# JinfengX/PointCloudPDF

Measured on AMD Instinct MI355X. Metric: points/sec fwd+bwd (PT-v1 Seg50 + PDF U-decoder, 100k-pt scenes), higher is better.
Workload: dtype f32

## Files before the change

### include/pdfops.h

```cpp
#ifndef PDFOPS_H
#define PDFOPS_H

#ifdef __cplusplus
extern "C" {
#endif

#define PDF_OK 0
#define PDF_ERR_BAD_ARG (-1)
#define PDF_ERR_NSAMPLE (-2)
#define PDF_ERR_UNSUPPORTED (-3)

#define PDF_ABI_VERSION 11
int pdf_abi_version(void);
const char *pdf_build_info(void);
int pdf_dist_fma_mode(void);
#define PDF_MMA_F32 0
#define PDF_MMA_F16 1
#define PDF_MMA_BF16 2

int pdf_knn_query(int m, int nsample, const float *xyz, const float *new_xyz,
                  const int *offset, const int *new_offset, int b,
                  int *idx, float *dist2, void *stream);

long pdf_knn_workspace_bytes(int b, int n, int m);
int pdf_knn_grid_supported(int nsample);
int pdf_knn_query_ws(int m, int nsample, int n, const float *xyz, const float *new_xyz, const int *offset,
                     const int *new_offset, int b, int *idx, float *dist2, void *workspace, long workspace_bytes,
                     void *stream);
int pdf_knn_grid_build(int n, const float *xyz, const int *offset, int b, void *workspace, long workspace_bytes, void *stream);
int pdf_knn_query_grid(int m, int nsample, int n, const float *xyz, const float *new_xyz, const int *offset, const int *new_offset, int b,
                       int *idx, float *dist2, void *workspace, long workspace_bytes, void *stream);
int pdf_knn_query_ws_counted(int m, int nsample, int n, const float *xyz, const float *new_xyz, const int *offset,
                             const int *new_offset, int b, int *idx, float *dist2, void *workspace, long workspace_bytes,
                             unsigned long long *pairs, void *stream);
int pdf_knn_query_list(int m, int nsample, const float *xyz, const float *new_xyz, const int *offset,
                       const int *new_offset, int b, int *idx, float *dist2, const int *qlist, const int *qcount,
                       void *stream);

int pdf_ball_query(int m, int nsample, float min_radius, float max_radius, const float *xyz, const float *new_xyz,
                   const int *offset, const int *new_offset, int b, int *idx, float *dist2, void *stream);

int pdf_random_ball_query(int m, int nsample, float min_radius, float max_radius, const int *order, const float *xyz,
                          const float *new_xyz, const int *offset, const int *new_offset, int b, int *idx, float *dist2,
                          void *stream);

int pdf_farthest_point_sampling(int b, int n, const float *xyz, const int *offset,
                                const int *new_offset, float *tmp, int *idx, void *stream);

int pdf_fps_reference_block_log2(int n);

long pdf_fps_workspace_bytes(int b, int n_total);
long pdf_fps_stats_offset(int b, int n_total);
int pdf_farthest_point_sampling_bucketed(int b, int n, int n_total, const float *xyz, const int *offset,
                                         const int *new_offset, void *workspace, long workspace_bytes,
                                         int *idx, void *stream);

int pdf_grouping_forward(int m, int nsample, int c, const float *input, const int *idx, float *output, void *stream);
int pdf_grouping_backward(int m, int nsample, int c, const float *grad_output, const int *idx, float *grad_input, void *stream);
int pdf_grouping_forward_ordered(int m, int nsample, int c, const float *input, const int *idx, const int *order, float *output, void *stream);
int pdf_group_forward_ordered(int m, int nsample, int c, int with_xyz, const float *feat, const float *xyz, const float *new_xyz,
                              const int *idx, const int *order, float *output, void *stream);
int pdf_interpolation_forward_ordered(int n, int c, int k, const float *input, const int *idx, const float *weight, const int *order,
                                      float *output, void *stream);
int pdf_subtraction_forward_ordered(int n, int nsample, int c, const float *input1, const float *input2, const int *idx, const int *order,
                                    float *output, void *stream);
int pdf_aggregation_forward_ordered(int n, int nsample, int c, int w_c, const float *input, const float *position, const float *weight,
                                    const int *idx, const int *order, float *output, void *stream);

int pdf_interpolation_forward(int n, int c, int k, const float *input, const int *idx, const float *weight, float *output, void *stream);
int pdf_interpolation_backward(int n, int c, int k, const float *grad_output, const int *idx, const float *weight, float *grad_input, void *stream);

int pdf_subtraction_forward(int n, int nsample, int c, const float *input1, const float *input2, const int *idx, float *output, void *stream);
int pdf_subtraction_backward(int n, int nsample, int c, const int *idx, const float *grad_output, float *grad_input1, float *grad_input2, void *stream);

int pdf_aggregation_forward(int n, int nsample, int c, int w_c, const float *input, const float *position,
                            const float *weight, const int *idx, float *output, void *stream);
int pdf_aggregation_backward(int n, int nsample, int c, int w_c, const float *input, const float *position,
                             const float *weight, const int *idx, const float *grad_output,
                             float *grad_input, float *grad_position, float *grad_weight, void *stream);

int pdf_attention_relation_step_forward(int m, int g, int c, const float *query, const float *key, const float *weight,
                                        const int *index_target, const int *index_refer, float *output, void *stream);
int pdf_attention_relation_step_backward(int m, int g, int c, const float *query, float *grad_query,
                                         const float *key, float *grad_key, const float *weight, float *grad_weight,
                                         const int *index_target, const int *index_refer, const float *grad_output, void *stream);
int pdf_attention_fusion_step_forward(int m, int g, int c, const float *weight, const float *value,
                                      const int *index_target, const int *index_refer, float *output, void *stream);
int pdf_attention_fusion_step_backward(int m, int g, int c, const float *weight, float *grad_weight,
                                       const float *value, float *grad_value,
                                       const int *index_target, const int *index_refer, const float *grad_output, void *stream);


int pdf_group_forward(int m, int nsample, int c, int with_xyz, const float *feat, const float *xyz,
                      const float *new_xyz, const int *idx, float *output, void *stream);
int pdf_group_backward(int m, int nsample, int c, int with_xyz, const float *grad_output, const int *idx,
                       float *grad_feat, void *stream);

int pdf_interpolation_weights(int n, int k, const float *dist2, float *weight, void *stream);

int pdf_pt_layer_supported(int nsample, int c);
long pdf_pt_layer_partial_floats(int n, int nsample, int c);
int pdf_pt_layer_forward(int n, int nsample, int c, const float *xq, const float *xk, const float *xv,
                         const float *p, const int *idx, const float *const *weights,
                         const float *const *bn_params, float *const *bn_buffers, int training, float eps,
                         float momentum, float *bn, float *saved, float *H, float *partial, float *out,
                         int storage_bf16, const int *order, void *stream);
int pdf_pt_layer_forward_m(int n, int nsample, int c, const float *xq, const float *xk, const float *xv,
                           const float *p, const int *idx, const float *const *weights,
                           const float *const *bn_params, float *const *bn_buffers, int training, float eps,
                           float momentum, float *bn, float *saved, float *H, float *partial, float *out,
                           int storage_bf16, const int *order, const double *moments, int *out_stat_rows, void *stream);

long pdf_pt_layer_bwd_partial_floats(int n, int nsample, int c);
long pdf_pt_layer_bwd_sums_floats(int c);
int pdf_pt_layer_backward(int n, int nsample, int c, const float *xq, const float *xk, const float *xv,
                          const float *p, const int *idx, const float *const *weights, const float *bn,
                          const float *saved, const float *H, const float *gout, float *gxq, float *gxk,
                          float *gxv, float *G2, float *G3, float *Wsm, float *GR, const int *inv_off, const int *inv_entry,
                          int entry_base, float *partial, float *sums, int storage_bf16, const int *order, const double *moments,
                          void *stream);

int pdf_bn_supported(int c);
long pdf_bn_partial_floats(long n, int c);
int pdf_bn_act_forward(long n, int c, const float *x, const float *res, const float *gamma, const float *beta,
                       float *running_mean, float *running_var, int training, float eps, float momentum, int relu,
                       float *coef, float *partial, float *y, void *stream);
int pdf_bn_act_backward(long n, int c, const float *gy, const float *x, const float *res, const float *coef,
                        int training, int relu, float *partial, float *sums, float *gx, float *gres, void *stream);
int pdf_bn_coef(long n, int c, const float *x, const float *gamma, const float *beta, float *running_mean,
                float *running_var, int training, float eps, float momentum, float *coef, float *partial, void *stream);
int pdf_bn_apply(long n, int c, const float *x, const float *res, const float *coef, int relu, float *y, void *stream);

long pdf_rowlin_partial_floats(long n, int o);
int pdf_rowlin_partial_rows(long n, int k, int o);
int pdf_rowlin_forward(long n, int k, int o, const float *x, long ldx, const float *w, int transpose_w,
                       const float *bias, const float *scale, const float *shift, int relu, float *y, long ldy,
                       int accumulate, float *partial, int mma_input, void *stream);
long pdf_rowlin_wgrad_ws_floats(long n, int k, int o, int ng);
int pdf_rowlin_wgrad(long n, int k, int o, const float *g, long ldg, const float *x, long ldx,
                     const float *scale, const float *shift, int relu, float *dw, float *db, float *ws, int mma_input, void *stream);
int pdf_bn_coef_from_partial(const float *partial, int rows, long n, int c, const float *gamma, const float *beta,
                             float *running_mean, float *running_var, float eps, float momentum, float *coef, void *stream);

int pdf_rowlin_multi(long n, int k, int o, int nin, int nout, const float *const *x, long ldx, const float *const *w,
                     int transpose_w, const float *const *bias, const float *scale, const float *shift, int relu,
                     float *const *y, long ldy, int accumulate, int mma_input, void *stream);
int pdf_rowlin_wgrad_multi(long n, int k, int o, int ng, const float *const *g, long ldg, const float *x, long ldx,
                           const float *scale, const float *shift, int relu, float *const *dw, float *const *db, float *ws, int mma_input, void *stream);
int pdf_rowlin_wgrad_group(long n, int k, int o, int ng, const float *const *g, long ldg, const float *const *x, long ldx,
                           const float *const *scale, const float *const *shift, const int *relu, float *const *dw,
                           float *const *db, float *ws, int mma_input, void *stream);

int pdf_kpconv_supported(int kp, int cin);
int pdf_kpconv_gather(int n, int m, int kp, int cin, const float *query, const float *support, const int *neighbors, const float *x,
                      const float *k_points, float extent, float *weighted, void *stream);
int pdf_kpconv_scatter(int n, int m, int kp, int cin, const float *query, const float *support, const int *neighbors,
                       const float *grad_weighted, const float *k_points, float extent, float *grad_x, void *stream);
int pdf_rowlin_dgrad_bstats(long n, int k, int o, int nin, const float *const *x, long ldx, const float *const *w, float *y, long ldy,
                            const float *bx, long ldb, const float *bcoef, int brelu, float *partial, int *partial_rows,
                            int mma_input, void *stream);
int pdf_rowlin_forward_bn(long n, int k, int o, const float *x, long ldx, const float *w, const float *bias, const float *scale,
                          const float *shift, int relu, float *y, long ldy, float *partial, const float *gamma, const float *beta,
                          float *running_mean, float *running_var, float eps, float momentum, float *coef, int mma_input, void *stream);
int pdf_bn_act_backward_presummed(long n, int c, const float *gy, const float *x, const float *coef, int training, int relu,
                                  const float *partial, int partial_rows, float *sums, float *gx, void *stream);

int pdf_bn_coef_eval_or_partial(const float *partial, int rows, long n, int c, const float *gamma, const float *beta,
                                float *running_mean, float *running_var, int training, float eps, float momentum,
                                float *coef, void *stream);
int pdf_block_pre_forward(long n, int c, void *const *p, int training, float eps, float momentum, int mma_input, void *stream);
int pdf_block_pre_backward(long n, int c, void *const *p, int training, int mma_input, void *stream);
int pdf_block_post_forward(long n, int c, void *const *p, int training, float eps, float momentum, int mma_input, void *stream);
int pdf_block_post_backward(long n, int c, void *const *p, int training, int mma_input, void *stream);
int pdf_bottleneck_forward(long n, int nsample, int c, void *const *p, int training, float eps, float momentum, int storage_bf16, int mma_input, void *stream);
int pdf_bottleneck_backward(long n, int nsample, int c, void *const *p, int training, int entry_base, int storage_bf16, int mma_input, void *stream);
int pdf_linbn_forward(long n, int k, int o, void *const *p, int training, int relu, float eps, float momentum, int mma_input, void *stream);
int pdf_linbn_backward(long n, int k, int o, void *const *p, int training, int relu, int mma_input, void *stream);

int pdf_rowlin_forward_roww(long n, int k, int o, const float *x, long ldx, const float *w, int transpose_w, float *y, long ldy,
                            int accumulate, const float *roww, long rws, int mma_input, void *stream);
int pdf_rowlin_wgrad_roww(long n, int k, int o, const float *g, long ldg, const float *x, long ldx, float *dw, const float *roww,
                          long rws, float *ws, int mma_input, void *stream);
int pdf_bn_bwd_sums(long n, int c, const float *gy, const float *x, const float *coef, int relu, float *partial, float *sums,
                    void *stream);

int pdf_td_supported(int nsample, int cin, int cout);
int pdf_td_tables(long m, int b, const float *p_src, const float *p_new, const int *idx, const int *new_offset, float *rel4, float *Z,
                  float *scene_sums, long n, const int *inv_off, const int *inv_entry, int entry_base,
                  void *stream);
long pdf_td_gram_floats(int cin);
long pdf_td_fwd_scratch_floats(long n, int cin);
long pdf_td_bwd_scratch_floats(long m, int cin, int cout);
int pdf_td_forward(long n, long m, int cin, int cout, void *const *p, int training, float eps, float momentum, int mma_input, void *stream);
int pdf_td_backward(long n, long m, int cin, int cout, void *const *p, int entry_base, int mma_input, void *stream);

int pdf_seg_sum_rows(long n, int c, const float *src, const int *inv_off, const int *inv_entry, int entry_base, float scale, float *out,
                     void *stream);
int pdf_seg_sum_rows_own(long n, int c, int nsample, const float *src, const int *inv_off, const int *inv_entry, int entry_base, float scale,
                         const int *order, float *out, float *out_own, void *stream);
int pdf_seg_sum_rows_strided(long n, int c, const float *src, long src_stride, const int *inv_off, const int *inv_entry, int entry_base,
                             float scale, float *out, void *stream);
int pdf_seg_sum_rows_x(long n, int c, const float *src, long src_stride, int src_bf16, const int *inv_off, const int *inv_entry, int entry_base,
                       float scale, float *out, void *stream);
int pdf_seg_sum_weighted_x(long n, int c, int nsample, int w_c, const float *src, const float *w, int w_bf16, const int *inv_off,
                           const int *inv_entry, int entry_base, const int *order, float *out, void *stream);
int pdf_seg_sum_weighted_ordered(long n, int c, int nsample, int w_c, const float *src, const float *w, const int *inv_off,
                                 const int *inv_entry, int entry_base, const int *order, float *out, void *stream);
int pdf_seg_sum_weighted(long n, int c, int nsample, int w_c, const float *src, const float *w, const int *inv_off, const int *inv_entry,
                         int entry_base, float *out, void *stream);

long pdf_ce_workspace_floats(void);
int pdf_ce_forward(long n, int c, const float *logits, const long *target, long ignore, float *grad, float *acc, float *loss,
                   void *stream);
int pdf_ce_backward(long n, int c, const float *dlogits, const float *acc, const float *gy, float *grad_out, void *stream);

long pdf_incr_kl_workspace_floats(void);
int pdf_incr_kl_forward(long n, int cs, int ct, const float *student, const float *teacher, const long *labels, long ignore, float inv_tp,
                        float inv_tt, float *grad, float *acc, float *loss, void *stream);
int pdf_incr_kl_backward(long n, int cs, const float *dgrad, const float *acc, const float *gy, float *grad_out, void *stream);

long pdf_lovasz_workspace_bytes(long n, int c);
int pdf_lovasz_forward(long n, int c, const float *logits, const long *target, long ignore, const unsigned char *class_mask, float *prob,
                       float *dlogits, float *loss, void *workspace, void *stream);
int pdf_lovasz_backward(long n, int c, const float *dlogits, const float *gy, float scale, float *grad_out, void *stream);

long pdf_openset_metrics_workspace_bytes(long n, int c);
int pdf_openset_metrics(long n, int c, const float *logits, const long *pred, const float *score, const long *target, long ignore,
                        const unsigned char *unknown, int k, long long *hist, double *record, void *workspace, void *stream);

long pdf_knn_rel_moments_ws_doubles(int b, long m);
int pdf_knn_rel_moments(int b, long n, int nsample, const float *xyz, const int *offset, const int *idx, double *out, double *ws, void *stream);
int pdf_knn_rel_moments_q(int b, long m, int nsample, const float *xyz, const float *new_xyz, const int *new_offset, const int *idx,
                          double *out, double *ws, void *stream);

int pdf_scene_morton_keys(long n, int b, const float *xyz, const int *offset, float *bounds, long long *keys, void *stream);

int pdf_sgd_chunk(void);
int pdf_sgd_step(int nchunks, const void *tab, const int *chunks, float lr, float momentum, float weight_decay, const float *found_inf,
                 void *stream);
int pdf_grad_unscale(int nchunks, const void *tab, const int *chunks, const float *inv_scale, float *found_inf, void *stream);
int pdf_scaler_update(float *scale, float *inv_scale, int *growth_tracker, float *found_inf, float growth_factor, float backoff_factor,
                      int growth_interval, void *stream);
int pdf_adam_step(int nchunks, int ntensors, const void *tab, const int *chunks, double lr, double beta1, double beta2, double eps,
                  double weight_decay, int decoupled, const float *found_inf, void *stream);
int pdf_adam_grad_unscale(int nchunks, const void *tab, const int *chunks, const float *inv_scale, float *found_inf, void *stream);

int pdf_attention_step1_forward_v2(int N, int M, int h, int C, unsigned n_max, const float *q, const float *k,
                                   const int *index0_offsets, const int *index1, float *attn, void *stream);
int pdf_attention_step1_backward_v2(int N, int M, int h, int C, unsigned n_max, const float *grad_out, const int *index0_offsets,
                                    const int *index1, const float *q, const float *k, float *grad_q, float *grad_k, void *stream);
int pdf_dot_prod_with_idx_forward_v3(int N, int M, int h, int hdim, unsigned n_max, const float *q, const int *index_q_offsets,
                                     const float *k, const int *index_k, const float *table_q, const float *table_k,
                                     const int *rel_idx, float *output, void *stream);
int pdf_dot_prod_with_idx_backward_v3(int N, int M, int h, int hdim, unsigned n_max, const float *grad_out, const float *q,
                                      const int *index_q_offsets, const float *k, const int *index_k, const float *table_q,
                                      const float *table_k, const int *rel_idx, float *grad_q, float *grad_k, float *grad_table_q,
                                      float *grad_table_k, void *stream);
int pdf_attention_step2_with_rel_pos_value_forward_v2(int N, int M, int h, int hdim, unsigned n_max, const float *attn, const float *v,
                                                      const int *index0_offsets, const int *index1, const float *table,
                                                      const int *rel_idx, float *output, void *stream);
// ... 145 lines not shown
```

### pointcloudpdf_amd/_native.py

```python
import ctypes
import os
import threading

import torch

_HERE = os.path.dirname(os.path.abspath(__file__))
DIST_FMA = int(os.environ.get("PDFOPS_DIST_FMA", "0") or 0)
if DIST_FMA not in (0, 1, 2):
    raise RuntimeError(f"PDFOPS_DIST_FMA={DIST_FMA}: expected 0 (as written), 1 or 2 (csrc/pdfops_common.h)")


def library_path(dist_fma=0):
    return os.path.join(_HERE, "lib", "libpdfops.so" if not dist_fma else f"libpdfops_fma{int(dist_fma)}.so")


LIB_PATH = library_path(DIST_FMA)
ABI_VERSION = 11

c_int = ctypes.c_int
c_long = ctypes.c_long
c_void_p = ctypes.c_void_p
c_float = ctypes.c_float
c_double = ctypes.c_double

_PROTOS = {
    "knn_query": "iippppipp",
    "ball_query": "iiffppppipp",
    "random_ball_query": "iiffpppppipp",
    "farthest_point_sampling": "iippppp",
    "grouping_forward": "iiippp",
    "grouping_backward": "iiippp",
    "interpolation_forward": "iiipppp",
    "interpolation_backward": "iiipppp",
    "subtraction_forward": "iiipppp",
    "subtraction_backward": "iiipppp",
    "aggregation_forward": "iiiippppp",
    "aggregation_backward": "iiiipppppppp",
    "attention_relation_step_forward": "iiipppppp",
    "attention_relation_step_backward": "iiippppppppp",
    "attention_fusion_step_forward": "iiippppp",
    "attention_fusion_step_backward": "iiippppppp",
    "attention_step1_forward_v2": "iiiiippppp",
    "attention_step1_backward_v2": "iiiiippppppp",
    "dot_prod_with_idx_forward_v3": "iiiiipppppppp",
    "dot_prod_with_idx_backward_v3": "iiiiipppppppppppp",
    "attention_step2_with_rel_pos_value_forward_v2": "iiiiippppppp",
    "attention_step2_with_rel_pos_value_backward_v2": "iiiiipppppppppp",
    "segment_softmax_forward": "iiippp",
    "segment_softmax_backward": "iiipppp",
}
_HIP_ONLY_PROTOS = {
    "grid_hash": "lippdddippp",
    "grid_hash_f64": "lippdddppp",
    "philox4x64": "llllp",
    "aug_bounds": "ippppp",
    "aug_points": "ilpipppppp",
    "aug_keys": "ilpplp",
    "aug_elastic_noise": "ilpplp",
    "aug_elastic_blur": "ilpppi",
    "aug_elastic_apply": "ilpppppdpp",
    "radius_neighbors_self": "iifppipppl",
    "radius_neighbors_self_adaptive": "iiffppippppl",
    "vote_accumulate": "lipppppp",
    "fragment_bounds": "lliiipppppp",
    "fragment_gather": "lliiipppppipppppppp",
    "fragment_vote": "lliiippppppppp",
    "graph_forest": "lipppppipppl",
    "gmm2_1d": "ipppidd",
    "dot_prod_with_idx_forward_v3_l": "iiiiipppppppp",
    "dot_prod_with_idx_backward_v3_l": "iiiiipppppppppppp",
    "attention_step2_with_rel_pos_value_backward_v2_l": "iiiiipppppppppp",
    "scene_sum_rows": "ipiplip",
    "scene_repeat_rows": "iplipip",
    "region_stats": "ippppifppp",
    "region_seeds": "ippppip",
    "region_grow": "ippipppipiipppp",
    "region_edges": "ipppppippppppppppppl",
    "sort_floats_dev": "ipppppp",
    "gmm2_weak_dev": "ippppppppidd",
    "region_mask": "ippppppp",
    "region_tree": "ippipppppppp",
    "graph_forest_dev": "lipppppippppl",
    "gmm2_1d_dev": "ippppidd",
    "graph_forest_batch_dev": "ippippppppipppl",
    "wa_segment_rows": "iiiipppppplfpplf",
    "wa_segment_rows_ordered": "iiiipppppplfpplfp",
    "wa_table_grad": "iiiippppplfpp",
    "wa_grad_attn": "iiiiiplppplppp",
    "wa_logits_forward": "iiiiipplfpppppp",
    "wa_permute_edges": "iippp",
    "wa_logits_forward_ordered": "iiiiipplfppppppp",
    "wa_grad_attn_ordered": "iiiiiplppplpppp",
    "window_keys": "ippippfippp",
    "window_edges_count": "ippipppppp",
    "window_edges_fill": "ipppppppffipppp",
    "group_forward": "iiiippppp",
    "group_backward": "iiiippp",
    "interpolation_weights": "iipp",
    "farthest_point_sampling_bucketed": "iiipppplp",
    "grouping_forward_ordered": "iiipppp",
# ... 478 lines not shown
        lib.pdf_fragment_bounds_ws_doubles.restype = c_long
        lib.pdf_fragment_bounds_ws_doubles.argtypes = [c_int]
        lib.pdf_abi_version.restype = c_int
        lib.pdf_build_info.restype = ctypes.c_char_p
        got = int(lib.pdf_abi_version())
        if got != ABI_VERSION:
            raise PdfOpsError(f"libpdfops ABI {got} != {ABI_VERSION} expected by pointcloudpdf_amd/_native.py (include/pdfops.h: PDF_ABI_VERSION): "
                              "stale library -- rebuild with `python -m pointcloudpdf_amd.build --force`")
        for nm in ("pre_forward", "post_forward"):
            f = getattr(lib, "pdf_block_" + nm)
            f.restype = c_int
            f.argtypes = [c_long, c_int, c_void_p, c_int, ctypes.c_float, ctypes.c_float, c_int, c_void_p]
        lib.pdf_td_tables.restype = c_int
        lib.pdf_td_tables.argtypes = [c_long, c_int, c_void_p, c_void_p, c_void_p, c_void_p, c_void_p, c_void_p, c_void_p, c_long, c_void_p, c_void_p,
                                      c_int, c_void_p]
        lib.pdf_td_supported.restype = c_int
        lib.pdf_td_supported.argtypes = [c_int, c_int, c_int]
        lib.pdf_td_gram_floats.restype = c_long
        lib.pdf_td_gram_floats.argtypes = [c_int]
        lib.pdf_td_fwd_scratch_floats.restype = c_long
        lib.pdf_td_fwd_scratch_floats.argtypes = [c_long, c_int]
        lib.pdf_td_bwd_scratch_floats.restype = c_long
        lib.pdf_td_bwd_scratch_floats.argtypes = [c_long, c_int, c_int]
        lib.pdf_td_forward.restype = c_int
        lib.pdf_td_forward.argtypes = [c_long, c_long, c_int, c_int, c_void_p, c_int, ctypes.c_float, ctypes.c_float, c_int, c_void_p]
        lib.pdf_td_backward.restype = c_int
        lib.pdf_td_backward.argtypes = [c_long, c_long, c_int, c_int, c_void_p, c_int, c_int, c_void_p]
        lib.pdf_ce_workspace_floats.restype = c_long
        lib.pdf_ce_workspace_floats.argtypes = []
        lib.pdf_ce_forward.restype = c_int
        lib.pdf_ce_forward.argtypes = [c_long, c_int, c_void_p, c_void_p, c_long, c_void_p, c_void_p, c_void_p, c_void_p]
        lib.pdf_ce_backward.restype = c_int
        lib.pdf_ce_backward.argtypes = [c_long, c_int, c_void_p, c_void_p, c_void_p, c_void_p, c_void_p]
        lib.pdf_incr_kl_workspace_floats.restype = c_long
        lib.pdf_incr_kl_workspace_floats.argtypes = []
        lib.pdf_incr_kl_forward.restype = c_int
        lib.pdf_incr_kl_forward.argtypes = [c_long, c_int, c_int, c_void_p, c_void_p, c_void_p, c_long, ctypes.c_float, ctypes.c_float,
                                            c_void_p, c_void_p, c_void_p, c_void_p]
        lib.pdf_incr_kl_backward.restype = c_int
        lib.pdf_incr_kl_backward.argtypes = [c_long, c_int, c_void_p, c_void_p, c_void_p, c_void_p, c_void_p]
        lib.pdf_lovasz_workspace_bytes.restype = c_long
        lib.pdf_lovasz_workspace_bytes.argtypes = [c_long, c_int]
        lib.pdf_lovasz_forward.restype = c_int
        lib.pdf_lovasz_forward.argtypes = [c_long, c_int, c_void_p, c_void_p, c_long, c_void_p, c_void_p, c_void_p, c_void_p, c_void_p, c_void_p]
        lib.pdf_lovasz_backward.restype = c_int
        lib.pdf_lovasz_backward.argtypes = [c_long, c_int, c_void_p, c_void_p, ctypes.c_float, c_void_p, c_void_p]
        lib.pdf_openset_metrics_workspace_bytes.restype = c_long
        lib.pdf_openset_metrics_workspace_bytes.argtypes = [c_long, c_int]
        lib.pdf_openset_metrics.restype = c_int
        lib.pdf_openset_metrics.argtypes = [c_long, c_int, c_void_p, c_void_p, c_void_p, c_void_p, c_long, c_void_p, c_int, c_void_p, c_void_p,
                                            c_void_p, c_void_p]
        lib.pdf_knn_rel_moments.restype = c_int
        lib.pdf_knn_rel_moments.argtypes = [c_int, c_long, c_int, c_void_p, c_void_p, c_void_p, c_void_p, c_void_p, c_void_p]
        lib.pdf_knn_rel_moments_ws_doubles.restype = c_long
        lib.pdf_knn_rel_moments_ws_doubles.argtypes = [c_int, c_long]
        lib.pdf_knn_rel_moments_q.restype = c_int
        lib.pdf_knn_rel_moments_q.argtypes = [c_int, c_long, c_int, c_void_p, c_void_p, c_void_p, c_void_p, c_void_p, c_void_p, c_void_p]
        class CopySeg(ctypes.Structure):
            _fields_ = [("src", c_void_p), ("dst", c_void_p), ("nbytes", c_long), ("src_offset", c_void_p), ("sub", c_void_p),
                        ("sub_const", c_int), ("src_elems", c_int)]

        self.CopySeg = CopySeg
        lib.pdf_stage_copy.restype = c_int
        lib.pdf_stage_copy.argtypes = [c_int, c_void_p, c_void_p]
        lib.pdf_scene_morton_keys.restype = c_int
        lib.pdf_scene_morton_keys.argtypes = [c_long, c_int, c_void_p, c_void_p, c_void_p, c_void_p, c_void_p]
        lib.pdf_sgd_chunk.restype = c_int
        lib.pdf_sgd_chunk.argtypes = []
        lib.pdf_sgd_step.restype = c_int
        lib.pdf_sgd_step.argtypes = [c_int, c_void_p, c_void_p, ctypes.c_float, ctypes.c_float, ctypes.c_float, c_void_p, c_void_p]
        lib.pdf_grad_unscale.restype = c_int
        lib.pdf_grad_unscale.argtypes = [c_int, c_void_p, c_void_p, c_void_p, c_void_p, c_void_p]
        lib.pdf_scaler_update.restype = c_int
        lib.pdf_scaler_update.argtypes = [c_void_p, c_void_p, c_void_p, c_void_p, ctypes.c_float, ctypes.c_float, c_int, c_void_p]
        lib.pdf_adam_step.restype = c_int
        lib.pdf_adam_step.argtypes = [c_int, c_int, c_void_p, c_void_p, ctypes.c_double, ctypes.c_double, ctypes.c_double, ctypes.c_double,
                                      ctypes.c_double, c_int, c_void_p, c_void_p]
        lib.pdf_adam_grad_unscale.restype = c_int
        lib.pdf_adam_grad_unscale.argtypes = [c_int, c_void_p, c_void_p, c_void_p, c_void_p, c_void_p]
        lib.pdf_linbn_forward.restype = c_int
        lib.pdf_linbn_forward.argtypes = [c_long, c_int, c_int, c_void_p, c_int, c_int, ctypes.c_float, ctypes.c_float, c_int, c_void_p]
        lib.pdf_linbn_backward.restype = c_int
        lib.pdf_linbn_backward.argtypes = [c_long, c_int, c_int, c_void_p, c_int, c_int, c_int, c_void_p]
        lib.pdf_bottleneck_forward.restype = c_int
        lib.pdf_bottleneck_forward.argtypes = [c_long, c_int, c_int, c_void_p, c_int, ctypes.c_float, ctypes.c_float, c_int, c_int, c_void_p]
        lib.pdf_bottleneck_backward.restype = c_int
        lib.pdf_bottleneck_backward.argtypes = [c_long, c_int, c_int, c_void_p, c_int, c_int, c_int, c_int, c_void_p]
        for nm in ("pre_backward", "post_backward"):
            f = getattr(lib, "pdf_block_" + nm)
            f.restype = c_int
            f.argtypes = [c_long, c_int, c_void_p, c_int, c_int, c_void_p]
        lib.pdf_rowlin_multi.restype = c_int
        lib.pdf_rowlin_multi.argtypes = [c_long, c_int, c_int, c_int, c_int, c_void_p, c_long, c_void_p, c_int, c_void_p, c_void_p, c_void_p,
                                         c_int, c_void_p, c_long, c_int, c_int, c_void_p]
        lib.pdf_kpconv_supported.restype = c_int
        lib.pdf_kpconv_supported.argtypes = [c_int, c_int]
        for nm in ("pdf_kpconv_gather", "pdf_kpconv_scatter"):
            f = getattr(lib, nm)
            f.restype = c_int
            f.argtypes = [c_int, c_int, c_int, c_int, c_void_p, c_void_p, c_void_p, c_void_p, c_void_p, ctypes.c_float, c_void_p, c_void_p]
        lib.pdf_rowlin_wgrad_group.restype = c_int
        lib.pdf_rowlin_wgrad_group.argtypes = [c_long, c_int, c_int, c_int, c_void_p, c_long, c_void_p, c_long, c_void_p, c_void_p, c_void_p,
                                               c_void_p, c_void_p, c_void_p, c_int, c_void_p]
        lib.pdf_rowlin_wgrad_multi.restype = c_int
        lib.pdf_rowlin_wgrad_multi.argtypes = [c_long, c_int, c_int, c_int, c_void_p, c_long, c_void_p, c_long, c_void_p, c_void_p, c_int,
                                               c_void_p, c_void_p, c_void_p, c_int, c_void_p]
        lib.pdf_rowlin_wgrad_ws_floats.restype = c_long
        lib.pdf_rowlin_wgrad_ws_floats.argtypes = [c_long, c_int, c_int, c_int]
        lib.pdf_rowlin_dgrad_bstats.restype = c_int
        lib.pdf_rowlin_dgrad_bstats.argtypes = [c_long, c_int, c_int, c_int, c_void_p, c_long, c_void_p, c_void_p, c_long, c_void_p, c_long,
                                                c_void_p, c_int, c_void_p, ctypes.POINTER(c_int), c_int, c_void_p]
        lib.pdf_bn_act_backward_presummed.restype = c_int
        lib.pdf_bn_act_backward_presummed.argtypes = [c_long, c_int, c_void_p, c_void_p, c_void_p, c_int, c_int, c_void_p, c_int, c_void_p,
                                                      c_void_p, c_void_p]
        lib.pdf_rowlin_partial_floats.restype = c_long
        lib.pdf_rowlin_partial_floats.argtypes = [c_long, c_int]
        lib.pdf_rowlin_partial_rows.restype = c_int
        lib.pdf_rowlin_partial_rows.argtypes = [c_long, c_int, c_int]
        lib.pdf_rowlin_forward.restype = c_int
        lib.pdf_rowlin_forward.argtypes = [c_long, c_int, c_int, c_void_p, c_long, c_void_p, c_int, c_void_p, c_void_p, c_void_p,
                                           c_int, c_void_p, c_long, c_int, c_void_p, c_int, c_void_p]
        lib.pdf_rowlin_wgrad.restype = c_int
        lib.pdf_rowlin_wgrad.argtypes = [c_long, c_int, c_int, c_void_p, c_long, c_void_p, c_long, c_void_p, c_void_p, c_int,
                                         c_void_p, c_void_p, c_void_p, c_int, c_void_p]
        lib.pdf_bn_coef_from_partial.restype = c_int
        lib.pdf_bn_coef_from_partial.argtypes = [c_void_p, c_int, c_long, c_int, c_void_p, c_void_p, c_void_p, c_void_p,
                                                 ctypes.c_float, ctypes.c_float, c_void_p, c_void_p]
        lib.pdf_bn_coef.restype = c_int
        lib.pdf_bn_coef.argtypes = [c_long, c_int, c_void_p, c_void_p, c_void_p, c_void_p, c_void_p, c_int, ctypes.c_float,
                                    ctypes.c_float, c_void_p, c_void_p, c_void_p]
        lib.pdf_bn_apply.restype = c_int
        lib.pdf_bn_apply.argtypes = [c_long, c_int, c_void_p, c_void_p, c_void_p, c_int, c_void_p, c_void_p]
        lib.pdf_bn_supported.restype = c_int
        lib.pdf_bn_supported.argtypes = [c_int]
        lib.pdf_bn_partial_floats.restype = c_long
        lib.pdf_bn_partial_floats.argtypes = [c_long, c_int]
        lib.pdf_bn_act_forward.restype = c_int
        lib.pdf_bn_act_forward.argtypes = [c_long, c_int] + [c_void_p] * 6 + [c_int, ctypes.c_float, ctypes.c_float, c_int] + [c_void_p] * 4
        lib.pdf_bn_act_backward.restype = c_int
        lib.pdf_bn_act_backward.argtypes = [c_long, c_int] + [c_void_p] * 4 + [c_int, c_int] + [c_void_p] * 5
        lib.pdf_pt_layer_supported.restype = c_int
        lib.pdf_pt_layer_supported.argtypes = [c_int, c_int]
        for fn in (lib.pdf_pt_layer_partial_floats, lib.pdf_pt_layer_bwd_partial_floats):
            fn.restype = c_long
            fn.argtypes = [c_int, c_int, c_int]
        lib.pdf_pt_layer_bwd_sums_floats.restype = c_long
        lib.pdf_pt_layer_bwd_sums_floats.argtypes = [c_int]
        lib.pdf_pt_layer_forward.restype = c_int
        lib.pdf_pt_layer_forward.argtypes = [c_int, c_int, c_int] + [c_void_p] * 8 + [c_int, ctypes.c_float, ctypes.c_float] + [c_void_p] * 5 + [c_int, c_void_p, c_void_p]
        lib.pdf_knn_grid_build.restype = c_int
        lib.pdf_knn_grid_build.argtypes = [c_int, c_void_p, c_void_p, c_int, c_void_p, c_long, c_void_p]
        lib.pdf_knn_query_grid.restype = c_int
        lib.pdf_knn_query_grid.argtypes = [c_int, c_int, c_int, c_void_p, c_void_p, c_void_p, c_void_p, c_int, c_void_p, c_void_p, c_void_p, c_long, c_void_p]
        lib.pdf_pt_layer_backward.restype = c_int
        lib.pdf_pt_layer_backward.argtypes = [c_int, c_int, c_int] + [c_void_p] * 19 + [c_int] + [c_void_p] * 2 + [c_int, c_void_p, c_void_p, c_void_p]
        self.fps_mode = os.environ.get("PDFOPS_FPS", "bucketed")
        self.knn_mode = os.environ.get("PDFOPS_KNN", "grid")
        lib.pdf_knn_workspace_bytes.restype = c_long
        lib.pdf_knn_workspace_bytes.argtypes = [c_int, c_int, c_int]
        lib.pdf_graph_forest_workspace_bytes.restype = c_long
        lib.pdf_region_grow_list_points.restype = c_long
        lib.pdf_region_grow_list_points.argtypes = []
        lib.pdf_graph_forest_workspace_bytes.argtypes = [c_long, c_long, c_long]
        lib.pdf_knn_grid_supported.restype = c_int
        lib.pdf_knn_grid_supported.argtypes = [c_int]
        lib.pdf_knn_query_ws.restype = c_int
# ... 1101 lines not shown
```

### pointcloudpdf_amd/dense.py

```python
import ctypes
import os
from ctypes import c_void_p

import torch

def _amp_fwd(fn):
    import functools

    from . import _native
    inner = torch.amp.custom_fwd(fn, device_type="cuda", cast_inputs=torch.float32)

    @functools.wraps(fn)
    def wrapped(ctx, *args, **kwargs):
        ctx._pdf_mma = _native.current_mma_input()
        return inner(ctx, *args, **kwargs)

    return wrapped


def _amp_bwd(fn):
    import functools

    from . import _native
    inner = torch.amp.custom_bwd(fn, device_type="cuda")
# ... 645 lines not shown
        bump_counters([mod.bn.num_batches_tracked])
    return out


def transition_down_ok(mod, x):
    if not (x.is_cuda and x.dtype == torch.float32 and x.dim() == 2 and x.is_contiguous() and type(mod.bn) is torch.nn.BatchNorm1d
            and mod.bn.affine and mod.bn.track_running_stats and mod.bn.momentum is not None and mod.linear.bias is None):
        return False
    if torch.is_grad_enabled() and not mod.training and any(p.requires_grad for p in mod.parameters()):
        return False
    return bool(_be().lib.pdf_td_supported(mod.nsample, x.shape[1], mod.linear.weight.shape[0]))


class _LinBnFn(torch.autograd.Function):
    @staticmethod
    @_amp_fwd
    def forward(ctx, lin, bn, relu, x, W, b, gamma, beta):
        be = _be()
        _rcd(x, W, gamma)
        lib = be.lib
        n, k = x.shape
        o = W.shape[0]
        training = bn.training
        e = lambda *shape: torch.empty(shape, dtype=torch.float32, device=x.device)
        z, coef, y = e(n, o), e(4 * o), e(n, o)
        partial = e(int(lib.pdf_rowlin_partial_floats(n, o)))
        ptrs = [x.data_ptr(), W.data_ptr(), b.data_ptr() if b is not None else None, gamma.data_ptr(), beta.data_ptr(),
                bn.running_mean.data_ptr(), bn.running_var.data_ptr(), z.data_ptr(), coef.data_ptr(), y.data_ptr(), partial.data_ptr()]
        rc = lib.pdf_linbn_forward(n, k, o, (c_void_p * len(ptrs))(*ptrs), int(training), int(relu), ctypes.c_float(bn.eps),
                                   ctypes.c_float(bn.momentum), _mma(), be._stream())
        if rc != 0:
            raise RuntimeError(f"pdf_linbn_forward failed with status {rc}")
        ctx.save_for_backward(x, z, coef, W)
        ctx.cfg = (training, relu, b is not None)
        return y

    @staticmethod
    @_amp_bwd
    def backward(ctx, gy):
        x, z, coef, W = ctx.saved_tensors
        training, relu, has_bias = ctx.cfg
        be = _be()
        lib = be.lib
        n, k = x.shape
        o = W.shape[0]
        e = lambda *shape: torch.empty(shape, dtype=torch.float32, device=x.device)
        need_gx = ctx.needs_input_grad[3]
        gx = e(n, k) if need_gx else None
        grads, gz = e(o * k + 3 * o), e(n, o)
        partial = e(int(lib.pdf_bn_partial_floats(n, o)))
        gy = gy.contiguous()
        ws = be.wgrad_workspace(n, k, o, 1, x.device)
        ptrs = [gy.data_ptr(), x.data_ptr(), z.data_ptr(), coef.data_ptr(), W.data_ptr(), gx.data_ptr() if need_gx else None, grads.data_ptr(),
                gz.data_ptr(), partial.data_ptr(), ws.data_ptr()]
        rc = lib.pdf_linbn_backward(n, k, o, (c_void_p * len(ptrs))(*ptrs), int(training), int(relu), _mma(), be._stream())
        if rc != 0:
            raise RuntimeError(f"pdf_linbn_backward failed with status {rc}")
        ok = o * k
        return (None, None, None, gx, grads[:ok].view(o, k), grads[ok:ok + o] if has_bias else None, grads[ok + 2 * o:ok + 3 * o], grads[ok + o:ok + 2 * o])


LINBN = True


def linbn_ok(lin, bn, x):
    if not LINBN:
        return False
    if not (x.is_cuda and x.dim() == 2 and x.dtype == torch.float32 and x.is_contiguous() and type(bn) is torch.nn.BatchNorm1d and bn.affine
            and bn.track_running_stats and bn.momentum is not None):
        return False
    k, o = lin.in_features, lin.out_features
    if k not in (32, 64, 128, 256, 512) or o % 16 or not _be().bn_supported(o):
        return False
    if torch.is_grad_enabled() and not bn.training and any(p.requires_grad for p in list(lin.parameters()) + list(bn.parameters())):
        return False
    return True


def linear_bn_act(lin, bn, x, relu):
    y = _LinBnFn.apply(lin, bn, relu, x, lin.weight, lin.bias, bn.weight, bn.bias)
    if bn.training:
        bump_counters([bn.num_batches_tracked])
    return y
```

### pointcloudpdf_amd/point_transformer.py

```python
import os

import torch

import torch.nn as nn
import torch.nn.functional as F

from . import _native, pointops
from . import dense
from .dense import _amp_bwd, _amp_fwd, bn_act as _bn_act, linear as _lin
from .geometry import Geometry, tag_of
from .registry import MODELS


def _seq(seq, x):
    mods = list(seq)
    i = 0
    while i < len(mods):
        m = mods[i]
        if (isinstance(m, nn.Linear) and i + 1 < len(mods) and isinstance(mods[i + 1], nn.BatchNorm1d) and x.dim() == 2
                and dense.linbn_ok(m, mods[i + 1], x)):
            relu = i + 2 < len(mods) and isinstance(mods[i + 2], nn.ReLU)
            x = dense.linear_bn_act(m, mods[i + 1], x, relu)
            i += 3 if relu else 2
            continue
# ... 183 lines not shown

    @staticmethod
    @_amp_fwd
    def forward(ctx, x, offset, sizes_host):
        be = _scene_rows_kernels(x)
        ctx.sizes, ctx.n = [int(v) for v in sizes_host], x.shape[0]
        if be is None:
            ctx.offset = None
            return torch.cat([ch.sum(0, True) / ch.shape[0] for ch in x.split(ctx.sizes, dim=0)], 0)
        x = x.contiguous()
        ctx.offset = offset = offset.int().contiguous()
        out = torch.empty((len(ctx.sizes), x.shape[1]), dtype=x.dtype, device=x.device)
        be._call("scene_sum_rows", len(ctx.sizes), offset, x.shape[1], x, x.shape[1], 1, out)
        return out

    @staticmethod
    @_amp_bwd
    def backward(ctx, g):
        if ctx.offset is None:
            return torch.cat([(g[i:i + 1] / n).expand(n, -1) for i, n in enumerate(ctx.sizes)], 0), None, None
        g = g.contiguous()
        out = torch.empty((ctx.n, g.shape[1]), dtype=g.dtype, device=g.device)
        _native.backend_for(g)._call("scene_repeat_rows", len(ctx.sizes), ctx.offset, ctx.n, g.shape[1], g, 1, out)
        return out, None, None


class _RowsPerScene(torch.autograd.Function):

    @staticmethod
    @_amp_fwd
    def forward(ctx, rows, offset, sizes_dev, sizes_host, total):
        ctx.sizes = [int(v) for v in sizes_host]
        be = _scene_rows_kernels(rows)
        if be is None:
            ctx.offset = None
            return torch.repeat_interleave(rows, sizes_dev, dim=0, output_size=total)
        rows = rows.contiguous()
        ctx.offset = offset = offset.int().contiguous()
        out = torch.empty((total, rows.shape[1]), dtype=rows.dtype, device=rows.device)
        be._call("scene_repeat_rows", len(ctx.sizes), offset, total, rows.shape[1], rows, 0, out)
        return out

    @staticmethod
    @_amp_bwd
    def backward(ctx, g):
        if ctx.offset is None:
            return torch.cat([ch.sum(0, keepdim=True) for ch in g.split(ctx.sizes, dim=0)], 0), None, None, None, None
        g = g.contiguous()
        out = torch.empty((len(ctx.sizes), g.shape[1]), dtype=g.dtype, device=g.device)
        _native.backend_for(g)._call("scene_sum_rows", len(ctx.sizes), ctx.offset, g.shape[1], g, g.shape[1], 0, out)
        return out, None, None, None, None


class TransitionUp(nn.Module):

    def __init__(self, in_planes, out_planes=None):
        super().__init__()
        if out_planes is None:
            self.linear1 = nn.Sequential(nn.Linear(2 * in_planes, in_planes), nn.BatchNorm1d(in_planes), nn.ReLU(inplace=True))
            self.linear2 = nn.Sequential(nn.Linear(in_planes, in_planes), nn.ReLU(inplace=True))
        else:
            self.linear1 = nn.Sequential(nn.Linear(out_planes, out_planes), nn.BatchNorm1d(out_planes), nn.ReLU(inplace=True))
            self.linear2 = nn.Sequential(nn.Linear(in_planes, out_planes), nn.BatchNorm1d(out_planes), nn.ReLU(inplace=True))

    @staticmethod
    def _scene_sizes(p, o):
        tag = tag_of(p)
        ends = tag[0].offset_host(tag[1]) if tag is not None else [int(v) for v in o.detach().cpu().tolist()]
        return [ends[0]] + [ends[i] - ends[i - 1] for i in range(1, len(ends))]

    def forward(self, pxo1, pxo2=None):
        if pxo2 is None:
            p, x, o = pxo1
            sizes = self._scene_sizes(p, o)
            means = _SceneMean.apply(x, o, sizes)
            ctx = _seq(self.linear2, means)
            tag = tag_of(p)
            sizes_dev = tag[0].sizes(tag[1]) if tag is not None else torch.diff(o.long(), prepend=o.new_zeros(1).long())
            rep = _RowsPerScene.apply(ctx, o, sizes_dev, sizes, x.shape[0])
            x = _seq(self.linear1, torch.cat((x, rep), 1))
        else:
            p1, x1, o1 = pxo1
            p2, x2, o2 = pxo2
            x = _seq(self.linear1, x1) + pointops.interpolation(p2, p1, _seq(self.linear2, x2), o2, o1)
        return x


class Bottleneck(nn.Module):

    expansion = 1

    def __init__(self, in_planes, planes, share_planes=8, nsample=16):
        super().__init__()
        self.linear1 = nn.Linear(in_planes, planes, bias=False)
        self.bn1 = nn.BatchNorm1d(planes)
        self.transformer = PointTransformerLayer(planes, planes, share_planes, nsample)
        self.bn2 = nn.BatchNorm1d(planes)
        self.linear3 = nn.Linear(planes, planes * self.expansion, bias=False)
        self.bn3 = nn.BatchNorm1d(planes * self.expansion)
        self.relu = nn.ReLU(inplace=True)

    def _apply(self, fn, *a, **kw):
        self.__dict__.pop("_pdf_params", None)
        return super()._apply(fn, *a, **kw)

    matrix_core = os.environ.get("PDFOPS_MATRIX_CORE", "1") != "0"

    def forward(self, pxo):
        p, x, o = pxo
        identity = x
        t = self.transformer
        if self.matrix_core and dense.fused_ok(x, self.bn1, self.bn2, self.bn3):
            return [p, dense.bottleneck(self, p, x, o), o]
        x = _bn_act(self.bn1, _lin(self.linear1, x), None, True)
        x = _bn_act(self.bn2, self.transformer([p, x, o]), None, True)
        x = _bn_act(self.bn3, _lin(self.linear3, x), identity, True)
        return [p, x, o]


class PointTransformerSeg(nn.Module):

    def __init__(self, block, blocks, in_channels=6, num_classes=13):
        super().__init__()
        self.in_channels = in_channels
        self.in_planes, planes = in_channels, [32, 64, 128, 256, 512]
        share_planes = 8
        stride, nsample = [1, 4, 4, 4, 4], [8, 16, 16, 16, 16]
        self.strides, self.nsamples = stride, nsample
        for i in range(5):
            setattr(self, f"enc{i + 1}", self._make_enc(block, planes[i], blocks[i], share_planes, stride[i], nsample[i]))
        for i in range(4, -1, -1):
            setattr(self, f"dec{i + 1}", self._make_dec(block, planes[i], 1, share_planes, nsample[i], is_head=(i == 4)))
        self.cls = nn.Sequential(
            nn.Linear(planes[0], planes[0]), nn.BatchNorm1d(planes[0]), nn.ReLU(inplace=True), nn.Linear(planes[0], num_classes)
        )
        self._last_geometry = None

    def _make_enc(self, block, planes, blocks, share_planes=8, stride=1, nsample=16):
        layers = [TransitionDown(self.in_planes, planes * block.expansion, stride, nsample)]
        self.in_planes = planes * block.expansion
        layers += [block(self.in_planes, self.in_planes, share_planes, nsample=nsample) for _ in range(blocks)]
        return nn.Sequential(*layers)

    def _make_dec(self, block, planes, blocks, share_planes=8, nsample=16, is_head=False):
        layers = [TransitionUp(self.in_planes, None if is_head else planes * block.expansion)]
        self.in_planes = planes * block.expansion
        layers += [block(self.in_planes, self.in_planes, share_planes, nsample=nsample) for _ in range(blocks)]
        return nn.Sequential(*layers)

    def geometry_for(self, data_dict):
        geom = data_dict.get("pdf_geometry") if isinstance(data_dict, dict) else None
        if geom is None:
            geom = Geometry(data_dict["coord"], data_dict["offset"], data_dict.get("offset_host"))
            try:
                data_dict["pdf_geometry"] = geom
            except TypeError:
                pass
        self._last_geometry = geom
        return geom

    @dense.fp32_path
    def forward(self, data_dict):
        geom = self.geometry_for(data_dict)
        p0, o0 = geom.coord(0), geom.offset(0)
        x0 = data_dict["feat"]
        if x0.dtype in (torch.float16, torch.bfloat16):
# ... 31 lines not shown
```

Measured before the change: 13.49 million.

## Fuse TransitionUp skip branch, interpolation and add into one join kernel

Adds a fused TransitionUp path. Both Linear+BN branches run their GEMMs with BN stats, then one HIP kernel applies BN+ReLU to each branch, does the 3-NN weighted interpolation of the coarse branch and adds the result to the fine branch in a single pass. This is meant to remove separate BN-activation, interpolation and elementwise-add kernels and their intermediate tensors. Backward reuses the existing linbn backward and interpolation backward. The new path is gated by an environment flag that defaults on and needs cached interpolation indices from the geometry tag.

```diff
diff --git a/include/pdfops.h b/include/pdfops.h
--- a/include/pdfops.h
+++ b/include/pdfops.h
@@ -10,7 +10,7 @@
 #define PDF_ERR_NSAMPLE (-2)
 #define PDF_ERR_UNSUPPORTED (-3)
 
-#define PDF_ABI_VERSION 11
+#define PDF_ABI_VERSION 12
 int pdf_abi_version(void);
 const char *pdf_build_info(void);
 int pdf_dist_fma_mode(void);
@@ -176,6 +176,11 @@
 int pdf_bottleneck_backward(long n, int nsample, int c, void *const *p, int training, int entry_base, int storage_bf16, int mma_input, void *stream);
 int pdf_linbn_forward(long n, int k, int o, void *const *p, int training, int relu, float eps, float momentum, int mma_input, void *stream);
 int pdf_linbn_backward(long n, int k, int o, void *const *p, int training, int relu, int mma_input, void *stream);
+int pdf_tu_supported(int o, int k);
+int pdf_tu_join_forward(long n, int o, const float *z1, const float *coef1, const float *z2, const float *coef2, const int *idx,
+                        const float *weight, const int *order, float *out, void *stream);
+int pdf_tu_forward(long n, long m, int k1, int k2, int o, void *const *p, int training, float eps1, float momentum1, float eps2,
+                   float momentum2, int mma_input, void *stream);
 
 int pdf_rowlin_forward_roww(long n, int k, int o, const float *x, long ldx, const float *w, int transpose_w, float *y, long ldy,
                             int accumulate, const float *roww, long rws, int mma_input, void *stream);
diff --git a/pointcloudpdf_amd/_native.py b/pointcloudpdf_amd/_native.py
--- a/pointcloudpdf_amd/_native.py
+++ b/pointcloudpdf_amd/_native.py
@@ -15,7 +15,7 @@
 
 
 LIB_PATH = library_path(DIST_FMA)
-ABI_VERSION = 11
+ABI_VERSION = 12
 
 c_int = ctypes.c_int
 c_long = ctypes.c_long
@@ -660,6 +660,12 @@
         lib.pdf_linbn_forward.argtypes = [c_long, c_int, c_int, c_void_p, c_int, c_int, ctypes.c_float, ctypes.c_float, c_int, c_void_p]
         lib.pdf_linbn_backward.restype = c_int
         lib.pdf_linbn_backward.argtypes = [c_long, c_int, c_int, c_void_p, c_int, c_int, c_int, c_void_p]
+        lib.pdf_tu_supported.restype = c_int
+        lib.pdf_tu_supported.argtypes = [c_int, c_int]
+        lib.pdf_tu_join_forward.restype = c_int
+        lib.pdf_tu_join_forward.argtypes = [c_long, c_int] + [c_void_p] * 9
+        lib.pdf_tu_forward.restype = c_int
+        lib.pdf_tu_forward.argtypes = [c_long, c_long, c_int, c_int, c_int, c_void_p, c_int] + [ctypes.c_float] * 4 + [c_int, c_void_p]
         lib.pdf_bottleneck_forward.restype = c_int
         lib.pdf_bottleneck_forward.argtypes = [c_long, c_int, c_int, c_void_p, c_int, ctypes.c_float, ctypes.c_float, c_int, c_int, c_void_p]
         lib.pdf_bottleneck_backward.restype = c_int
diff --git a/pointcloudpdf_amd/csrc/transition_up.hip b/pointcloudpdf_amd/csrc/transition_up.hip
--- /dev/null
+++ b/pointcloudpdf_amd/csrc/transition_up.hip
@@ -0,0 +1,98 @@
+#include "pdfops_common.h"
+
+namespace tu {
+
+constexpr int TB = 256;
+constexpr int FR = 4;
+
+typedef float v4f __attribute__((ext_vector_type(4)));
+
+__device__ __forceinline__ v4f relu4(v4f v) { return __builtin_elementwise_max(v, (v4f)(0.f)); }
+
+static inline bool width_ok(int o) { return o == 32 || o == 64 || o == 128 || o == 256 || o == 512; }
+static inline int log2i(int v) { int s = 0; while ((1 << s) < v) ++s; return s; }
+
+__global__ __launch_bounds__(TB) void k_join_fwd(unsigned n, int lg , const int *__restrict__ order, const v4f *__restrict__ z1,
+                                                 const v4f *__restrict__ coef1, const v4f *__restrict__ z2, const v4f *__restrict__ coef2,
+                                                 const int *__restrict__ idx, const float *__restrict__ weight, v4f *__restrict__ out) {
+    const unsigned cv = 1u << lg, rpb = TB >> lg, col = threadIdx.x & (cv - 1), tr = threadIdx.x >> lg;
+    const unsigned first = pdf_xcd_chunked_block(blockIdx.x, gridDim.x) * rpb * FR + tr;
+    if (first >= n) return;
+    const v4f s1 = coef1[col], t1 = coef1[cv + col], s2 = coef2[col], t2 = coef2[cv + col];
+    unsigned r[FR];
+    bool live[FR];
+    int j[FR][3];
+    float w[FR][3];
+    v4f a[FR], v[FR][3];
+#pragma unroll
+    for (int u = 0; u < FR; ++u) {
+        const unsigned sq = first + u * rpb;
+        live[u] = sq < n;
+        r[u] = order ? (unsigned)order[min(sq, n - 1)] : min(sq, n - 1);
+    }
+#pragma unroll
+    for (int u = 0; u < FR; ++u)
+#pragma unroll
+        for (int i = 0; i < 3; ++i) { j[u][i] = idx[(size_t)r[u] * 3 + i]; w[u][i] = weight[(size_t)r[u] * 3 + i]; }
+#pragma unroll
+    for (int u = 0; u < FR; ++u) {
+        a[u] = z1[(size_t)r[u] * cv + col];
+#pragma unroll
+        for (int i = 0; i < 3; ++i) v[u][i] = z2[(size_t)max(j[u][i], 0) * cv + col];
+    }
+#pragma unroll
+    for (int u = 0; u < FR; ++u) {
+        const v4f y1 = relu4(a[u] * s1 + t1);
+        v4f acc = (v4f)(0.f);
+#pragma unroll
+        for (int i = 0; i < 3; ++i) acc += (j[u][i] >= 0 ? relu4(v[u][i] * s2 + t2) : (v4f)(0.f)) * w[u][i];
+        if (live[u]) __builtin_nontemporal_store(y1 + acc, out + (size_t)r[u] * cv + col);
+    }
+}
+
+struct Err {
+    int rc = 0;
+    Err &operator<<(int r) { if (rc == 0 && r != 0) rc = r; return *this; }
+};
+
+}
+
+extern "C" int pdf_tu_supported(int o, int k) { return tu::width_ok(o) && k == 3; }
+
+extern "C" int pdf_tu_join_forward(long n, int o, const float *z1, const float *coef1, const float *z2, const float *coef2, const int *idx,
+                                   const float *weight, const int *order, float *out, void *stream) {
+    if (n == 0) return PDF_OK;
+    if (n < 0 || !z1 || !coef1 || !z2 || !coef2 || !idx || !weight || !out) return PDF_ERR_BAD_ARG;
+    if (!tu::width_ok(o) || n * 3 >= (1L << 31)) return PDF_ERR_UNSUPPORTED;
+    const int lg = tu::log2i(o / 4);
+    const long span = (long)(tu::TB >> lg) * tu::FR;
+    tu::k_join_fwd<<<(unsigned)((n + span - 1) / span), tu::TB, 0, static_cast<hipStream_t>(stream)>>>(
+        (unsigned)n, lg, order, (const tu::v4f *)z1, (const tu::v4f *)coef1, (const tu::v4f *)z2, (const tu::v4f *)coef2, idx, weight, (tu::v4f *)out);
+    return pdf_launch_status();
+}
+
+extern "C" int pdf_tu_forward(long n, long m, int k1, int k2, int o, void *const *p, int training, float eps1, float momentum1, float eps2,
+                              float momentum2, int mma_input, void *stream) {
+    if (n < 1 || m < 1 || !p) return PDF_ERR_BAD_ARG;
+    if (!tu::width_ok(o) || !pdf_bn_supported(o)) return PDF_ERR_UNSUPPORTED;
+    tu::Err e;
+    const long rows[2] = {n, m};
+    const int ks[2] = {k1, k2};
+    const float eps[2] = {eps1, eps2}, mom[2] = {momentum1, momentum2};
+    for (int b = 0; b < 2; ++b) {
+        void *const *q = p + 10 * b;
+        float *z = (float *)q[7], *coef = (float *)q[8], *partial = (float *)q[9];
+        if (training) {
+            e << pdf_rowlin_forward_bn(rows[b], ks[b], o, (const float *)q[0], ks[b], (const float *)q[1], (const float *)q[2], nullptr, nullptr, 0, z, o,
+                                       partial, (const float *)q[3], (const float *)q[4], (float *)q[5], (float *)q[6], eps[b], mom[b], coef, mma_input, stream);
+        } else {
+            e << pdf_rowlin_forward(rows[b], ks[b], o, (const float *)q[0], ks[b], (const float *)q[1], 0, (const float *)q[2], nullptr, nullptr, 0, z, o, 0,
+                                    nullptr, mma_input, stream);
+            e << pdf_bn_coef_eval_or_partial(partial, 0, rows[b], o, (const float *)q[3], (const float *)q[4], (float *)q[5], (float *)q[6], 0, eps[b],
+                                             mom[b], coef, stream);
+        }
+    }
+    if (e.rc) return e.rc;
+    return pdf_tu_join_forward(n, o, (const float *)p[7], (const float *)p[8], (const float *)p[17], (const float *)p[18], (const int *)p[20],
+                               (const float *)p[21], (const int *)p[22], (float *)p[23], stream);
+}
diff --git a/pointcloudpdf_amd/dense.py b/pointcloudpdf_amd/dense.py
--- a/pointcloudpdf_amd/dense.py
+++ b/pointcloudpdf_amd/dense.py
@@ -751,3 +751,93 @@
     if bn.training:
         bump_counters([bn.num_batches_tracked])
     return y
+
+
+class _TransitionUpFn(torch.autograd.Function):
+    @staticmethod
+    @_amp_fwd
+    def forward(ctx, bn1, bn2, idx, weight, x1, x2, W1, b1, g1, be1, W2, b2, g2, be2):
+        from . import _native
+        be = _be()
+        _rcd(x1, x2, W1, W2, idx, weight)
+        lib = be.lib
+        n, k1 = x1.shape
+        m, k2 = x2.shape
+        o = W1.shape[0]
+        training = bn1.training
+        e = lambda *shape: torch.empty(shape, dtype=torch.float32, device=x1.device)
+        z1, coef1, z2, coef2, out = e(n, o), e(4 * o), e(m, o), e(4 * o), e(n, o)
+        part1, part2 = e(int(lib.pdf_rowlin_partial_floats(n, o))), e(int(lib.pdf_rowlin_partial_floats(m, o)))
+        order = _native.order_of(idx)
+        P = lambda t: None if t is None else t.data_ptr()
+        ptrs = [P(x1), P(W1), P(b1), P(g1), P(be1), P(bn1.running_mean), P(bn1.running_var), P(z1), P(coef1), P(part1),
+                P(x2), P(W2), P(b2), P(g2), P(be2), P(bn2.running_mean), P(bn2.running_var), P(z2), P(coef2), P(part2),
+                P(idx), P(weight), P(order), P(out)]
+        rc = lib.pdf_tu_forward(n, m, k1, k2, o, (c_void_p * len(ptrs))(*ptrs), int(training), ctypes.c_float(bn1.eps), ctypes.c_float(bn1.momentum),
+                                ctypes.c_float(bn2.eps), ctypes.c_float(bn2.momentum), _mma(), be._stream())
+        if rc != 0:
+            raise RuntimeError(f"pdf_tu_forward failed with status {rc}")
+        ctx.save_for_backward(x1, x2, z1, z2, coef1, coef2, idx, weight, W1, W2)
+        ctx.cfg = (training, b1 is not None, b2 is not None)
+        return out
+
+    @staticmethod
+    @_amp_bwd
+    def backward(ctx, g):
+        from . import _native
+        x1, x2, z1, z2, coef1, coef2, idx, weight, W1, W2 = ctx.saved_tensors
+        training, has_b1, has_b2 = ctx.cfg
+        be = _be()
+        lib = be.lib
+        n, k1 = x1.shape
+        m, k2 = x2.shape
+        o = W1.shape[0]
+        e = lambda *shape: torch.empty(shape, dtype=torch.float32, device=g.device)
+        g = g.contiguous()
+        P = lambda t: None if t is None else t.data_ptr()
+        gx1 = e(n, k1) if ctx.needs_input_grad[4] else None
+        grads1, gz1 = e(o * k1 + 3 * o), e(n, o)
+        ptrs = [P(g), P(x1), P(z1), P(coef1), P(W1), P(gx1), P(grads1), P(gz1), P(e(int(lib.pdf_bn_partial_floats(n, o)))),
+                P(be.wgrad_workspace(n, k1, o, 1, g.device))]
+        rc = lib.pdf_linbn_backward(n, k1, o, (c_void_p * len(ptrs))(*ptrs), int(training), 1, _mma(), be._stream())
+        if rc != 0:
+            raise RuntimeError(f"pdf_linbn_backward failed with status {rc}")
+        gx2 = e(m, k2) if ctx.needs_input_grad[5] else None
+        grads2, gz2 = e(o * k2 + 3 * o), e(m, o)
+        ws2 = be.wgrad_workspace(m, k2, o, 1, g.device)
+        gy2 = be.interpolation_backward(g, idx, weight, m)
+        ptrs = [P(gy2), P(x2), P(z2), P(coef2), P(W2), P(gx2), P(grads2), P(gz2), P(e(int(lib.pdf_bn_partial_floats(m, o)))), P(ws2)]
+        rc = lib.pdf_linbn_backward(m, k2, o, (c_void_p * len(ptrs))(*ptrs), int(training), 1, _mma(), be._stream())
+        if rc != 0:
+            raise RuntimeError(f"pdf_linbn_backward failed with status {rc}")
+        ok1, ok2 = o * k1, o * k2
+        return (None, None, None, None, gx1, gx2,
+                grads1[:ok1].view(o, k1), grads1[ok1:ok1 + o] if has_b1 else None, grads1[ok1 + 2 * o:ok1 + 3 * o], grads1[ok1 + o:ok1 + 2 * o],
+                grads2[:ok2].view(o, k2), grads2[ok2:ok2 + o] if has_b2 else None, grads2[ok2 + 2 * o:ok2 + 3 * o], grads2[ok2 + o:ok2 + 2 * o])
+
+
+TU_JOIN = os.environ.get("PDFOPS_TU_JOIN", "1") != "0"
+
+
+def transition_up_ok(mod, x1, x2, idx, weight):
+    if not TU_JOIN:
+        return False
+    s1, s2 = list(mod.linear1), list(mod.linear2)
+    for s in (s1, s2):
+        if not (len(s) == 3 and isinstance(s[0], nn.Linear) and isinstance(s[1], nn.BatchNorm1d) and isinstance(s[2], nn.ReLU)):
+            return False
+    if not (linbn_ok(s1[0], s1[1], x1) and linbn_ok(s2[0], s2[1], x2)) or s1[1].training != s2[1].training:
+        return False
+    o = s1[0].out_features
+    if s2[0].out_features != o or not _be().lib.pdf_tu_supported(o, idx.shape[1]):
+        return False
+    return (idx.dtype == torch.int32 and idx.is_contiguous() and idx.shape[0] == x1.shape[0] and weight.dtype == torch.float32
+            and weight.is_contiguous() and weight.shape == idx.shape and idx.device == x1.device and x2.device == x1.device)
+
+
+def transition_up(mod, x1, x2, idx, weight):
+    (l1, bn1, _), (l2, bn2, _) = list(mod.linear1), list(mod.linear2)
+    out = _TransitionUpFn.apply(bn1, bn2, idx, weight, x1, x2, l1.weight, l1.bias, bn1.weight, bn1.bias, l2.weight, l2.bias, bn2.weight, bn2.bias)
+    if bn1.training:
+        bump_counters([bn1.num_batches_tracked, bn2.num_batches_tracked])
+    return out
diff --git a/pointcloudpdf_amd/point_transformer.py b/pointcloudpdf_amd/point_transformer.py
--- a/pointcloudpdf_amd/point_transformer.py
+++ b/pointcloudpdf_amd/point_transformer.py
@@ -289,6 +289,12 @@
         else:
             p1, x1, o1 = pxo1
             p2, x2, o2 = pxo2
+            tc, tf = tag_of(p2), tag_of(p1)
+            if (tc is not None and tf is not None and tc[0] is tf[0] and x1.dim() == 2 and x2.dim() == 2 and x1.shape[0] == p1.shape[0]
+                    and x2.shape[0] == p2.shape[0]):
+                idx, weight = tc[0].interp(tc[1], tf[1], 3)
+                if dense.transition_up_ok(self, x1, x2, idx, weight):
+                    return dense.transition_up(self, x1, x2, idx, weight)
             x = _seq(self.linear1, x1) + pointops.interpolation(p2, p1, _seq(self.linear2, x2), o2, o1)
         return x
 
```

Result: no change. 13.53 million (median of 4 runs) (+0.3%).
